# GloireLINVANI/3D_Gaussian_Splatting_Project

Hardware: AMD Instinct MI355X
Metric: Gaussians·views/sec labelled (3M G, 1080p), majority vote; first vote_view submit -> labels on the host (higher is better)
Workload: dtype f64

## Files before the change

### 3d_gaussian_splatting_project_amd/csrc/gsx_ctx.hpp

```cpp
#pragma once
#include <hip/hip_runtime.h>

#include <chrono>
#include <cstdarg>
#include <cstdint>
#include <cstdio>
#include <map>
#include <cstddef>
#include <string>
#include <vector>

#include "../../include/gsx.h"
#include "host_pack.hpp"

namespace gsx {

void set_global_error(const char* fmt, ...);
struct Ctx;
int fail(Ctx* c, int code, const char* fmt, ...);

#define GSX_HIP(ctx, call)                                                                         \
    do {                                                                                           \
        hipError_t e__ = (call);                                                                   \
        if (e__ != hipSuccess)                                                                     \
// ... 166 lines not shown
    long long compact_bytes = 0;
    void* h_labels = nullptr;
    size_t h_labels_cap = 0;
    hipEvent_t h_ev[kLabelChunks] = {nullptr, nullptr, nullptr, nullptr};
    void* h_views = nullptr;
    size_t h_views_cap = 0;
    hipEvent_t h_views_ev = nullptr;
    std::vector<ViewDesc> own_views;
    int own_first_view = 0;
    const void* pool_base = nullptr;
    int n_flushed = 0;
    bool planes_valid = false;
    bool planes_zero = false;
    bool planes_stale = false;
    DevBuf cnt, fv;
    DevBuf keys, labels;
    DevBuf labels8;
    DevBuf bcnt, bcodes;
    DevBuf cand, codes;
    bool labels_valid = false;
    int opt_filter_project = 1;
    int opt_early_vote = 1;
    int opt_early_at = 0;
    std::chrono::steady_clock::time_point early_t0;
    int opt_early_replay = 1;
    bool early_replayed = false;
    int early_state = 0;
    int early_done = 0;
    int early_batches = 0;
    hipStream_t stream2 = nullptr;
    bool stream_borrowed = false;
    int opt_render_share_stream = 1;
    bool early_inflight = false;
    hipEvent_t early_maps_ev = nullptr, early_done_ev = nullptr, early_up_ev = nullptr;
    DevBuf ecnt, efv;
    DevBuf erec;
    DevBuf e_views, e_cull;
    void* h_early = nullptr;
    size_t h_early_cap = 0;

    int64_t rn = 0;
    DevBuf r_order, r_buffer, r_tex;
    DevBuf r_sh;
    DevBuf r_fdc, r_shc;
    bool r_sh_valid = false, r_sh_on = false;
    int r_sh_deg = 0;
    DevBuf r_labels, r_edit_code, r_edit_tab, r_edit_hidden;
    bool r_edits_on = false;
    int64_t r_edit_hidden_n = 0;
    DevBuf r_image;
    int r_W = 0, r_H = 0;
    DevBuf r_ranges, r_small, r_scan;
    DevBuf r_depth, r_bucket, r_rect, r_count, r_offset, r_rec;
    DevBuf r_pre;
    struct PreSet {
        DevBuf depth, rect, rec, pre;
    };
    static constexpr int kPreSets = 3;
    PreSet r_sets[kPreSets];
    DevBuf r_pre_args;
    std::vector<unsigned long long> r_pre_args_host;
    hipEvent_t r_pre_ev[kPreSets] = {nullptr, nullptr, nullptr};
    int r_pre_ext = -1;
    int opt_render_multi_pre = 1;
    DevBuf r_keys0, r_keys1, r_vals0, r_vals1;
    DevBuf r_tile_order;
    int r_sorted_in = 0;
// ... 109 lines not shown
```

### 3d_gaussian_splatting_project_amd/csrc/vote.hip

```cpp
#include <hip/hip_runtime.h>

#include <chrono>
#include <cmath>

#include <algorithm>
#include <cmath>
#include <cstdlib>
#include <cstring>
#include <new>

#include <type_traits>

#ifndef GSX_ABLATE
#define GSX_ABLATE 0
#endif
#if GSX_ABLATE && !defined(GSX_EXPERIMENTS)
#error "GSX_ABLATE variants are experiments: build them with -DGSX_EXPERIMENTS (make experiments), never into libgsx.so"
#endif

#include "gsx_ctx.hpp"

namespace gsx {

static constexpr int kBlock = 256;
// ... 619 lines not shown
                    int c = old[u] + 1;
#pragma unroll
                    for (int w = 0; w < u; ++w) c += (bin[w] == bin[u]) ? 1 : 0;
                    h[bin[u]] = (uint8_t)c;
                    if (c >= bestc) {
                        bestc = c;
                        best = bin[u];
                    }
                }
            }
        } else {
#pragma unroll
            for (int u = 0; u < U; ++u) {
                if (bin[u] >= 0) {
                    const int c = h[bin[u]] + 1;
                    h[bin[u]] = (uint8_t)c;
                    if (c >= bestc) {
                        bestc = c;
                        best = bin[u];
                    }
                }
            }
        }
        };
    int vb = p.nviews;
    for (; vb >= U; vb -= U) chunk(std::true_type{}, vb);
    if (vb > 0) chunk(std::false_type{}, vb);
    if (valid) {
        const long long o = p.perm ? (long long)p.perm[i] : i;
        labels[o] = best - 1 + (best < 0);
    }
}

template <int U, int DIV>
__global__ __launch_bounds__(kBlock) void vote_record_kernel(FusedParams p, const ViewDesc* __restrict__ views,
                                                             uint8_t* __restrict__ rec) {
    const long long i = (long long)logical_block(blockIdx.x, gridDim.x, p.xcd_swizzle) * kBlock + threadIdx.x;
    const bool valid = i < p.n;
    const long long ic = valid ? i : 0;
    const float xf = p.x[ic], yf = p.y[ic], zf = p.z[ic];
    const double X = valid ? (double)xf : __builtin_nan("");
    const double Y = valid ? (double)yf : 0.0;
    const double Z = valid ? (double)zf : 0.0;
    const uint8_t* __restrict__ pool = p.pool;
    const int lane = threadIdx.x & 63;
    uint8_t* r = rec + (i - lane) * p.nviews + lane;
    const CullMasks cmask = wave_cull_masks(p.cull, p.cull_pitch, p.nviews, X, Y, Z, p.cull_tally);
    auto chunk = [&](auto full, int vb) {
        constexpr bool kFull = decltype(full)::value;
        int bin[U];
        gather_chunk<U, DIV, kFull>(views, pool, vb, X, Y, Z, cull_bits<U>(cmask, p.nviews - vb), bin, p.filt_h);
#pragma unroll
        for (int u = 0; u < U; ++u)
            if (kFull || vb - 1 - u >= 0) r[(vb - 1 - u) * 64] = (uint8_t)(bin[u] + 1);
    };
    int vb = p.nviews;
    for (; vb >= U; vb -= U) chunk(std::true_type{}, vb);
    if (vb > 0) chunk(std::false_type{}, vb);
}

template <int U, int DIV>
__global__ __launch_bounds__(kBlock) void vote_fused_replay_kernel(FusedParams p, const ViewDesc* __restrict__ views,
                                                                   const uint8_t* __restrict__ rec, int E,
                                                                   int* __restrict__ labels) {
    extern __shared__ uint32_t lds[];
    uint32_t* row = lds + threadIdx.x * p.stride_dw;
    uint8_t* h = reinterpret_cast<uint8_t*>(row);
    for (int k = 0; k < p.stride_dw; ++k) row[k] = 0;
    const long long i = (long long)logical_block(blockIdx.x, gridDim.x, p.xcd_swizzle) * kBlock + threadIdx.x;
    const bool valid = i < p.n;
    const long long ic = valid ? i : 0;
    const float xf = p.x[ic], yf = p.y[ic], zf = p.z[ic];
    const double X = valid ? (double)xf : __builtin_nan("");
    const double Y = valid ? (double)yf : 0.0;
    const double Z = valid ? (double)zf : 0.0;
    const uint8_t* __restrict__ pool = p.pool;
    int best = -1, bestc = 0;
    auto vote = [&](int b) {
        const int c = h[b] + 1;
        h[b] = (uint8_t)c;
        if (c >= bestc) {
            bestc = c;
            best = b;
        }
    };
    const CullMasks cmask = wave_cull_masks(p.cull, p.cull_pitch, p.nviews, X, Y, Z, p.cull_tally);
    auto chunk = [&](auto full, int vb) {
        constexpr bool kFull = decltype(full)::value;
        int bin[U];
        gather_chunk<U, DIV, kFull>(views, pool, vb, X, Y, Z, cull_bits<U>(cmask, p.nviews - vb), bin, p.filt_h);
#pragma unroll
        for (int u = 0; u < U; ++u)
            if (bin[u] >= 0) vote(bin[u]);
    };
    int vb = p.nviews;
    for (; vb >= U; vb -= U) chunk(std::true_type{}, vb);
    if (vb > 0) chunk(std::false_type{}, vb);
    constexpr int kReplay = 16;
    const int lane = threadIdx.x & 63;
    const uint8_t* __restrict__ r = rec + (i - lane) * E + lane;
    for (int v0 = E; v0 > 0; v0 -= kReplay) {
        unsigned b[kReplay];
#pragma unroll
        for (int j = 0; j < kReplay; ++j) {
            const int v = v0 - 1 - j;
            const unsigned got = r[max(v, 0) * 64];
            b[j] = v >= 0 ? got : 0u;
        }
#pragma unroll
        for (int j = 0; j < kReplay; ++j)
            if (b[j]) vote((int)b[j] - 1);
    }
    if (valid) {
        const long long o = p.perm ? (long long)p.perm[i] : i;
        labels[o] = best - 1 + (best < 0);
    }
}

typedef unsigned short u16x2 __attribute__((ext_vector_type(2)));
__device__ __forceinline__ uint32_t pk_max_u16(uint32_t a, uint32_t b) {
    return __builtin_bit_cast(uint32_t, __builtin_elementwise_max(__builtin_bit_cast(u16x2, a), __builtin_bit_cast(u16x2, b)));
}

template <int U, int DIV, int NQ>
__global__ __launch_bounds__(kBlock, 4) void vote_fused_final_kernel(FusedParams p, const ViewDesc* __restrict__ views,
                                                                     const uint8_t* __restrict__ cntA,
                                                                     const uint8_t* __restrict__ fvA,
                                                                     const uint8_t* __restrict__ recA, int E,
                                                                     int* __restrict__ labels, int ablate_arg) {
#ifdef GSX_EXPERIMENTS
    const int ablate = ablate_arg;
#else
    constexpr int ablate = 0;
#endif
    extern __shared__ uint32_t lds[];
    const long long i = (long long)logical_block(blockIdx.x, gridDim.x, p.xcd_swizzle) * kBlock + threadIdx.x;
    const bool valid = i < p.n;
    const long long ic = valid ? i : 0;
    const float xf = p.x[ic], yf = p.y[ic], zf = p.z[ic];
    const double X = valid ? (double)xf : __builtin_nan("");
    const double Y = valid ? (double)yf : 0.0;
    const double Z = valid ? (double)zf : 0.0;
    const uint8_t* __restrict__ pool = p.pool;
    const int lane = threadIdx.x & 63;
    const int g = lane >> 4;
    const int nq = (p.bins + 3) >> 2;
    uint32_t* wl = lds + (threadIdx.x >> 6) * (nq * 64);
// ... 492 lines not shown
    if (n_classes < 1 || n_classes > 255)
        return fail(c, GSX_E_UNSUPPORTED, "vote_begin: n_classes=%d outside [1,255] (u8 seg maps)", n_classes);
    if (first_view < 0 || total_views < 1 || total_views > 65535 || first_view >= total_views)
        return fail(c, GSX_E_INVALID, "vote_begin: first_view=%d total_views=%d (need 0 <= first < total <= 65535)",
                    first_view, total_views);
    GSX_HIP(c, hipSetDevice(c->device));
    c->n_classes = n_classes;
    c->bins = n_classes + 1;
    c->first_view = first_view;
    c->total_views = total_views;
    c->local_codes = c->opt_local_codes != 0;
    c->wide = total_views > 255 && !c->local_codes;
    c->slabs = c->opt_slabs > 0 ? c->opt_slabs : 1;
    c->sn = ((c->n + c->slabs - 1) / c->slabs + 255) / 256 * 256;
    if (c->sn == 0) c->sn = 256;
    c->n_pad = c->sn * c->slabs;
    c->views.clear();
    c->pend_count = 0;
    c->compact_bytes = 0;
    c->views_dirty = true;
    c->pool_base = nullptr;
    c->seg_used = 0;
    c->n_flushed = 0;
    c->planes_valid = false;
    c->planes_zero = false;
    c->planes_stale = false;
    c->labels_valid = false;
    {
        const int rcj = early_join(c);
        if (rcj) return rcj;
    }
    c->early_state = 0;
    c->early_done = 0;
    c->early_batches = 0;
    GSX_HIP(c, c->errflag.ensure(sizeof(int)));
    GSX_HIP(c, hipMemsetAsync(c->errflag.p, 0x7f, sizeof(int), c->stream));
    c->vote_begun = true;
    return GSX_OK;
}

static int pool_reserve(Ctx* c, size_t need) {
    if (need <= c->segpool.cap) return GSX_OK;
    {
        const int rcf = vote_flush_pending(c);
        if (rcf) return rcf;
    }
    if (c->early_state == 1 || c->early_batches > 0) {
        GSX_HIP(c, hipStreamSynchronize(c->stream2));
        c->early_inflight = false;
        c->early_state = -1;
        c->early_batches = 0;
    }
    size_t cap = c->segpool.cap ? c->segpool.cap : ((size_t)64 << 20);
    while (cap < need) cap *= 2;
    void* np = nullptr;
    GSX_HIP(c, hipMalloc(&np, cap));
    if (c->seg_used) {
        hipError_t e = hipMemcpyAsync(np, c->segpool.p, c->seg_used, hipMemcpyDeviceToDevice, c->stream);
        if (e == hipSuccess) e = hipStreamSynchronize(c->stream);
        if (e != hipSuccess) {
            (void)hipFree(np);
            return fail(c, GSX_E_HIP, "seg pool growth copy failed: %s", hipGetErrorString(e));
        }
    }
    c->segpool.release();
    c->segpool.p = np;
// ... 27 lines not shown
        const size_t all = stride * (size_t)(c->total_views - c->first_view);
        need = std::max(need, std::min(all, (size_t)32 << 30));
    }
    return pool_reserve(c, need);
}

static void push_view(Ctx* c, const gsx_camera* cam, const MapLayout& L, size_t off, int img_w, int img_h) {
    ViewDesc vd;
    fill_view_desc(vd, cam, L.w, L.h, img_w, img_h);
    vd.seg_off = (long long)off;
    vd.seg_row_bytes = L.strip_bytes;
    vd.coarse_row_bytes = L.cstrip_bytes;
    vd.coarse_delta = (unsigned)L.coarse_off;
    c->views.push_back(vd);
    c->views_dirty = true;
    c->seg_used = off + L.map_bytes;
    c->labels_valid = false;
}

static void launch_pack(Ctx* c, const PackArgs& a, int jobs, int seg_dtype, bool vec, long long cells);

static Workers* host_workers(Ctx* c, const void* near = nullptr) {
    if (!c->workers) {
        try {
            c->workers = new Workers(c->opt_host_threads > 0 ? c->opt_host_threads : default_host_threads(), numa_node_of(near));
        } catch (...) {
            c->workers = nullptr;
        }
    }
    return c->workers;
}

static int early_vote_stage(Ctx* c);

static int vote_view_host(Ctx* c, const gsx_camera* cam, const void* seg, int seg_dtype, int seg_w, int seg_h, int img_w, int img_h) {
    MapLayout L;
    int rc = view_prologue(c, "vote_view", cam, seg, 1, seg_dtype, seg_w, seg_h, img_w, img_h, L);
    if (rc) return rc;
    if (c->opt_host_pack) {
        const size_t stride = (L.map_bytes + 255) / 256 * 256;
        constexpr int kSlots = kDmaBatch * kDmaGroups;
        const bool compact = c->opt_host_compact && L.strip_bytes && L.cstrip_bytes;
        const CompactLayout CL = compact ? compact_layout(L) : CompactLayout{};
        const size_t slot_bytes = compact ? (CL.capacity + 255) / 256 * 256 : stride;
        if (c->hring_slot != slot_bytes || !c->hring || c->hring_compact != compact) {
            if ((rc = vote_flush_pending(c))) return rc;
            for (int g = 0; g < kDmaGroups; ++g) {
                if (c->hring_busy[g]) GSX_HIP(c, hipEventSynchronize(c->hring_ev[g]));
                c->hring_busy[g] = false;
                if (!c->hring_ev[g]) GSX_HIP(c, hipEventCreateWithFlags(&c->hring_ev[g], hipEventDisableTiming));
            }
            if (c->hring_bytes < slot_bytes * kSlots) {
                if (c->hring) GSX_HIP(c, hipHostFree(c->hring));
                c->hring = nullptr;
                c->hring_bytes = 0;
                GSX_HIP(c, hipHostMalloc(&c->hring, slot_bytes * kSlots, hipHostMallocDefault));
                c->hring_bytes = slot_bytes * kSlots;
            }
            if (!compact) std::memset(c->hring, 0, slot_bytes * kSlots);
            c->hring_slot = slot_bytes;
            c->hring_compact = compact;
            c->hring_next = 0;
            c->cgrp = 0;
            c->grp_recs = 0;
        }
        const size_t off = (c->seg_used + 255) / 256 * 256;
// ... 85 lines not shown
        const size_t raw = esz * (size_t)seg_w * (size_t)seg_h;
        if (slot.cap < raw) {
            GSX_HIP(c, hipHostFree(slot.p));
            slot.p = nullptr;
            slot.cap = 0;
            GSX_HIP(c, hipHostMalloc(&slot.p, raw, hipHostMallocDefault));
            slot.cap = raw;
        }
        DevBuf& land = c->dstage[c->ring_next];
        GSX_HIP(c, land.ensure(raw));
        host_copy(host_workers(c, seg), slot.p, seg, raw);
        GSX_HIP(c, hipMemcpyAsync(land.p, slot.p, raw, hipMemcpyHostToDevice, c->stream));
        const size_t off = (c->seg_used + 255) / 256 * 256;
        PackArgs a{};
        a.src[0] = land.p;
        a.dst[0] = c->segpool.as<uint8_t>() + off;
        a.view[0] = c->first_view + (int)c->views.size();
        a.w = L.w, a.h = L.h, a.strip_bytes = L.strip_bytes, a.cstrip_bytes = L.cstrip_bytes, a.cw = L.cw, a.ch = L.ch;
        a.bins = c->bins;
        a.coarse_off = (unsigned)L.coarse_off;
        a.err = c->errflag.as<int>();
        launch_pack(c, a, 1, seg_dtype, seg_w % 4 == 0, (long long)L.cw * L.ch);
        GSX_HIP(c, hipGetLastError());
        GSX_HIP(c, hipEventRecord(slot.ev, c->stream));
        slot.busy = true;
        c->ring_next = (c->ring_next + 1) % kPinSlots;
        push_view(c, cam, L, off, img_w, img_h);
        return GSX_OK;
    }
    return GSX_OK;
}

int vote_view(Ctx* c, const gsx_camera* cam, const void* seg, int seg_dtype, int seg_w, int seg_h, int img_w, int img_h) {
    const int rc = vote_view_host(c, cam, seg, seg_dtype, seg_w, seg_h, img_w, img_h);
    return rc ? rc : early_vote_stage(c);
}

static void launch_pack(Ctx* c, const PackArgs& a, int jobs, int seg_dtype, bool vec, long long cells) {
    using K = void (*)(PackArgs);
    static const K table[4][2] = {{seg_pack_fused_kernel<int32_t, 1, false>, seg_pack_fused_kernel<int32_t, 1, true>},
                                  {seg_pack_fused_kernel<int64_t, 1, false>, seg_pack_fused_kernel<int64_t, 1, true>},
                                  {seg_pack_fused_kernel<uint8_t, 0, false>, seg_pack_fused_kernel<uint8_t, 0, true>},
                                  {seg_pack_fused_kernel<uint8_t, 1, false>, seg_pack_fused_kernel<uint8_t, 1, true>}};
    ProfScope ps(c, "seg_pack");
    hipLaunchKernelGGL(table[seg_dtype][vec ? 1 : 0], dim3(grid_for(cells), jobs), dim3(kBlock), 0, c->stream, a);
}

int vote_views_device(Ctx* c, int n, const gsx_camera* cams, const void* const* segs, int seg_dtype, int seg_w, int seg_h,
                      int img_w, int img_h) {
    if (n <= 0) return n == 0 ? GSX_OK : fail(c, GSX_E_INVALID, "vote_views_device: n < 0");
    MapLayout L;
    int rc = view_prologue(c, "vote_views_device", cams, segs, n, seg_dtype, seg_w, seg_h, img_w, img_h, L);
    if (rc) return rc;
    for (int i = 0; i < n; ++i)
        if (!segs[i]) return fail(c, GSX_E_INVALID, "vote_views_device: map %d is NULL", i);
    const size_t esz = seg_dtype == GSX_SEG_I32 ? 4 : seg_dtype == GSX_SEG_I64 ? 8 : 1;
    const long long cells = (long long)L.cw * L.ch;
    for (int i0 = 0; i0 < n; i0 += kPackBatch) {
        const int m = std::min(kPackBatch, n - i0);
        PackArgs a{};
        bool vec = seg_w % 4 == 0;
        size_t off = 0;
        for (int k = 0; k < m; ++k) {
            off = (c->seg_used + 255) / 256 * 256;
            a.src[k] = segs[i0 + k];
            a.dst[k] = c->segpool.as<uint8_t>() + off;
            a.view[k] = c->first_view + (int)c->views.size();
            vec = vec && reinterpret_cast<uintptr_t>(segs[i0 + k]) % (4 * esz) == 0;
// ... 66 lines not shown
    }
    for (DevBuf& b : c->dstage) b.release();
    for (hipEvent_t& e : c->hring_ev) {
        if (e) (void)hipEventDestroy(e);
        e = nullptr;
    }
    if (c->hring) (void)hipHostFree(c->hring);
    c->hring = nullptr;
    c->hring_bytes = c->hring_slot = 0;
    std::free(c->h_scratch);
    c->h_scratch = nullptr;
    c->h_scratch_cap = 0;
    c->cstage.release();
    c->pend_count = 0;
    for (hipEvent_t& e : c->h_ev) {
        if (e) (void)hipEventDestroy(e);
        e = nullptr;
    }
    if (c->h_labels) (void)hipHostFree(c->h_labels);
    c->h_labels = nullptr;
    c->h_labels_cap = 0;
    if (c->h_views_ev) (void)hipEventDestroy(c->h_views_ev);
    c->h_views_ev = nullptr;
    if (c->h_views) (void)hipHostFree(c->h_views);
    c->h_views = nullptr;
    c->h_views_cap = 0;
    delete c->workers;
    c->workers = nullptr;
    if (c->stream2) {
        (void)hipStreamSynchronize(c->stream2);
        (void)hipStreamDestroy(c->stream2);
        c->stream2 = nullptr;
    }
    for (hipEvent_t* e : {&c->early_maps_ev, &c->early_done_ev, &c->early_up_ev}) {
        if (*e) (void)hipEventDestroy(*e);
        *e = nullptr;
    }
    if (c->h_early) (void)hipHostFree(c->h_early);
    c->h_early = nullptr;
    c->h_early_cap = 0;
    for (DevBuf* b : {&c->ecnt, &c->efv, &c->erec, &c->e_views, &c->e_cull}) b->release();
    c->early_state = -1;
}

int debug_host_pack(const void* seg, int seg_dtype, int w, int h, int n_classes, int tiled, int coarse, int threads,
                    uint8_t* out, int64_t out_cap, int64_t* bytes, int64_t* coarse_off, int32_t* bad) {
    if (!seg || w < 1 || h < 1 || w > 65535 || h > 65535 || n_classes < 1 || n_classes > 255 || seg_dtype < 0 || seg_dtype > 3)
        return fail(nullptr, GSX_E_INVALID, "debug_host_pack: bad arguments");
    const MapLayout L = map_layout(w, h, tiled != 0, coarse != 0 && n_classes + 1 <= 255);
    if (bytes) *bytes = (int64_t)L.map_bytes;
    if (coarse_off) *coarse_off = L.cstrip_bytes ? (int64_t)L.coarse_off : -1;
    if (!out) return GSX_OK;
    if (out_cap < (int64_t)L.map_bytes) return fail(nullptr, GSX_E_INVALID, "debug_host_pack: output buffer too small");
    Workers pool(threads > 0 ? threads : 1);
    const int b = host_pack_map(&pool, seg, seg_dtype, L, n_classes + 1, out);
    if (bad) *bad = b;
    return GSX_OK;
}

int debug_host_pack_compact(const void* seg, int seg_dtype, int w, int h, int n_classes, int threads, uint8_t* out, int64_t out_cap,
                            int64_t* bytes, int64_t* table_bytes, int64_t* stream_off, int32_t* bad) {
    if (!seg || w < 1 || h < 1 || w > 65535 || h > 65535 || n_classes < 1 || n_classes > 254 || seg_dtype < 0 || seg_dtype > 3 || !bytes)
        return fail(nullptr, GSX_E_INVALID, "debug_host_pack_compact: bad arguments");
    const MapLayout L = map_layout(w, h, true, true);
    const CompactLayout CL = compact_layout(L);
    if (table_bytes) *table_bytes = (int64_t)CL.table_bytes;
    if (stream_off) *stream_off = (int64_t)CL.stream_off;
    *bytes = (int64_t)CL.capacity;
    if (!out) return GSX_OK;
    if (out_cap < (int64_t)CL.capacity) return fail(nullptr, GSX_E_INVALID, "debug_host_pack_compact: output buffer too small");
    void* scratch = std::aligned_alloc(4096, (L.fine_bytes + 4095) / 4096 * 4096);
    if (!scratch) return fail(nullptr, GSX_E_HIP, "debug_host_pack_compact: out of memory");
    Workers pool(threads > 0 ? threads : 1);
    size_t blocks = 0;
// ... 228 lines not shown
static constexpr long long kEarlyMinGaussians = 1 << 18;
static constexpr int kEarlyMinViews = 32;
static constexpr double kEarlyUsPerGaussianView = 4.4e-6;
static constexpr double kRecordUsPerGaussianView = 1.7e-6;
static constexpr size_t kEarlySlack = 64 * 260;
static constexpr size_t kEarlyCullDoubles = (size_t)kCullStride * kCullPlanes * kEarlyPitch;

static bool early_common(const Ctx* c) {
    return c->opt_early_vote && c->first_view == 0 && !c->local_codes && c->slabs == 1 && c->n_flushed == 0 && !c->pool_base &&
           c->opt_flat_project && c->n > 0 && c->bins <= 255 &&
           (c->opt_early_vote == 2 || (c->n >= kEarlyMinGaussians && c->total_views >= kEarlyMinViews));
}
static bool early_possible(const Ctx* c) { return early_common(c) && c->total_views <= kMaxBatch && !c->wide; }
static bool early_batched_possible(const Ctx* c) { return early_common(c) && c->total_views > kMaxBatch && c->opt_batched_counts; }
static int early_batch_stage(Ctx* c);
static int early_batch_count(int total) {
    const int tail = std::min(std::max(total / 16, 16), 64), body = total - tail;
    return (body + kMaxBatch - 1) / kMaxBatch + 1;
}
static void early_batch_bounds(int total, int s, int& lo, int& hi) {
    const int tail = std::min(std::max(total / 16, 16), 64), body = total - tail;
    const int Sb = (body + kMaxBatch - 1) / kMaxBatch;
    if (s >= Sb) {
        lo = body;
        hi = total;
    } else {
        lo = (int)((long long)body * s / Sb);
        hi = (int)((long long)body * (s + 1) / Sb);
    }
}

static int early_upload(Ctx* c, int lo, int hi, int block, int blocks, hipStream_t st, int* dm) {
    const size_t vbytes = sizeof(ViewDesc) * kEarlyPitch, cbytes = sizeof(double) * kEarlyCullDoubles;
    if (!c->h_early) {
        GSX_HIP(c, hipHostMalloc(&c->h_early, vbytes + cbytes, hipHostMallocDefault));
        c->h_early_cap = vbytes + cbytes;
    }
    GSX_HIP(c, c->e_views.ensure(sizeof(ViewDesc) * (size_t)std::max(kEarlyPitch, c->total_views)));
    GSX_HIP(c, c->e_cull.ensure(cbytes * (size_t)std::max(2, blocks)));
    if (!c->early_up_ev) GSX_HIP(c, hipEventCreateWithFlags(&c->early_up_ev, hipEventDisableTiming));
    else GSX_HIP(c, hipEventSynchronize(c->early_up_ev));
    ViewDesc* hv = static_cast<ViewDesc*>(c->h_early);
    double* planes = reinterpret_cast<double*>(static_cast<char*>(c->h_early) + vbytes);
    std::memset(planes, 0, cbytes);
    const long long base = (long long)reinterpret_cast<uintptr_t>(c->segpool.p);
    bool simple = true, coarse = true;
    for (int i = lo; i < hi; ++i) {
        ViewDesc& v = hv[i - lo];
        v = c->views[i];
        v.seg_off += base;
        simple = simple && v.unit_scale && v.seg_row_bytes;
        coarse = coarse && v.coarse_row_bytes;
        double pl[kCullStride * kCullPlanes];
        cull_planes(v, pl);
        for (int k = 0; k < kCullStride * kCullPlanes; ++k) planes[(size_t)k * kEarlyPitch + (i - lo)] = pl[k];
    }
    *dm = !simple ? kDivFlat : (coarse && c->opt_seg_coarse ? (c->opt_filter_project ? kDivFiltCoarse : kDivFlatCoarse) : kDivFlatSimple);
    if (hi > lo) GSX_HIP(c, hipMemcpyAsync(c->e_views.as<ViewDesc>() + lo, hv, sizeof(ViewDesc) * (size_t)(hi - lo), hipMemcpyHostToDevice, st));
    GSX_HIP(c, hipMemcpyAsync(c->e_cull.as<double>() + (size_t)block * kEarlyCullDoubles, planes, cbytes, hipMemcpyHostToDevice, st));
    GSX_HIP(c, hipEventRecord(c->early_up_ev, st));
    return GSX_OK;
}

static FusedParams early_params(Ctx* c, int lo, int hi, int block, int stride_bytes_per_bin) {
    FusedParams p = fused_params(c, stride_bytes_per_bin);
    p.views = c->e_views.as<ViewDesc>() + lo;
    p.nviews = hi - lo;
    p.cull = c->opt_wave_cull ? c->e_cull.as<double>() + (size_t)block * kEarlyCullDoubles : nullptr;
    p.cull_pitch = kEarlyPitch;
    return p;
}

int early_join(Ctx* c) {
    if (!c->early_inflight) return GSX_OK;
    GSX_HIP(c, hipStreamWaitEvent(c->stream, c->early_done_ev, 0));
    c->early_inflight = false;
    return GSX_OK;
}

int second_stream(Ctx* c) {
    if (c->stream2) return GSX_OK;
    int least = 0, greatest = 0;
    GSX_HIP(c, hipDeviceGetStreamPriorityRange(&least, &greatest));
    GSX_HIP(c, hipStreamCreateWithPriority(&c->stream2, hipStreamNonBlocking, least));
    return GSX_OK;
}

static int early_streams(Ctx* c) {
    const int rc = second_stream(c);
    if (rc) return rc;
    if (!c->early_maps_ev) GSX_HIP(c, hipEventCreateWithFlags(&c->early_maps_ev, hipEventDisableTiming));
    if (!c->early_done_ev) GSX_HIP(c, hipEventCreateWithFlags(&c->early_done_ev, hipEventDisableTiming));
    return GSX_OK;
}

static int early_vote_stage(Ctx* c) {
    if (c->early_state == 0 && early_batched_possible(c)) return early_batch_stage(c);
    if (c->early_state != 0 || !early_possible(c)) return GSX_OK;
    const int nv = (int)c->views.size();
    int at;
    if (c->opt_early_at > 0) {
        at = std::max(1, (int)(((long long)c->total_views * c->opt_early_at + 999) / 1000));
        if (nv != at) return GSX_OK;
    } else {
        const auto now = std::chrono::steady_clock::now();
        if (nv == 1) c->early_t0 = now;
        if (nv < std::max(8, c->total_views / 4)) return GSX_OK;
        const double t_map = std::chrono::duration<double, std::micro>(now - c->early_t0).count() / (double)(nv - 1);
        const double t_view = (c->opt_early_replay ? kRecordUsPerGaussianView : kEarlyUsPerGaussianView) * (double)c->n;
        const int lo = (c->total_views + 1) / 2, hi = (int)(((long long)c->total_views * 880) / 1000);
        const int want = std::min(std::max((int)std::ceil(c->total_views * t_map / (t_map + t_view)), lo), std::max(lo, hi));
        if (nv < want) return GSX_OK;
        at = nv;
    }
    if (at >= c->total_views) return GSX_OK;
    int rc = vote_flush_pending(c);
    if (rc) return rc;
    if ((rc = early_streams(c))) return rc;
    const size_t plane = (size_t)c->bins * (size_t)c->n_pad;
    if (!c->opt_early_replay) {
        GSX_HIP(c, c->ecnt.ensure(plane + kEarlySlack));
        GSX_HIP(c, c->efv.ensure(plane + kEarlySlack));
    }
    GSX_HIP(c, c->erec.ensure((size_t)c->n_pad * (size_t)at));
    if ((rc = ensure_tally(c))) return rc;
    GSX_HIP(c, hipEventRecord(c->early_maps_ev, c->stream));
    GSX_HIP(c, hipStreamWaitEvent(c->stream2, c->early_maps_ev, 0));
    int dm = kDivFlat;
    if ((rc = early_upload(c, 0, at, 0, 2, c->stream2, &dm))) return rc;
    if (c->opt_early_replay) {
        FusedParams p = early_params(c, 0, at, 0, 1);
        auto kr = dm == kDivFiltCoarse ? vote_record_kernel<kUnroll, kDivFiltCoarse>
                 : dm == kDivFlatCoarse ? vote_record_kernel<kUnroll, kDivFlatCoarse>
                  : dm == kDivFlatSimple ? vote_record_kernel<kUnroll, kDivFlatSimple>
                                         : vote_record_kernel<kUnroll, kDivFlat>;
        {
            ProfScope ps(c, "vote_early_record", c->stream2);
            hipLaunchKernelGGL(kr, dim3(grid_for(c->n)), dim3(kBlock), 0, c->stream2, p, p.views, c->erec.as<uint8_t>());
            GSX_HIP(c, hipGetLastError());
        }
        GSX_HIP(c, hipEventRecord(c->early_done_ev, c->stream2));
        c->early_inflight = true;
        c->early_done = at;
        c->early_state = 1;
        c->early_replayed = true;
        return GSX_OK;
    }
    c->early_replayed = false;
    FusedParams p = early_params(c, 0, at, 0, 2);
    const size_t lds = (size_t)kBlock * p.stride_dw * 4;
    auto k = dm == kDivFiltCoarse ? vote_fused_planes_kernel<kUnroll, uint8_t, kDivFiltCoarse>
                 : dm == kDivFlatCoarse ? vote_fused_planes_kernel<kUnroll, uint8_t, kDivFlatCoarse>
             : dm == kDivFlatSimple ? vote_fused_planes_kernel<kUnroll, uint8_t, kDivFlatSimple>
                                    : vote_fused_planes_kernel<kUnroll, uint8_t, kDivFlat>;
    if ((rc = set_lds(c, k, lds))) return rc;
    {
        ProfScope ps(c, "vote_early_planes", c->stream2);
        hipLaunchKernelGGL(k, dim3(grid_for(c->n)), dim3(kBlock), lds, c->stream2, p, p.views, c->ecnt.as<uint8_t>(), c->efv.as<uint8_t>(),
                           64LL, 0, 1, 0, c->erec.as<uint8_t>());
        GSX_HIP(c, hipGetLastError());
    }
    GSX_HIP(c, hipEventRecord(c->early_done_ev, c->stream2));
    c->early_inflight = true;
    c->early_done = at;
    c->early_state = 1;
    return GSX_OK;
}

static int early_batch_stage(Ctx* c) {
    const int nv = (int)c->views.size();
    const int S = early_batch_count(c->total_views);
    const int s = c->early_batches;
    if (s >= S - 1) return GSX_OK;
// ... 4 lines not shown
    if (rc) return rc;
    if ((rc = early_streams(c))) return rc;
    const size_t plane = (size_t)c->bins * (size_t)c->n_pad;
    GSX_HIP(c, c->bcnt.ensure(plane * S));
    if ((rc = ensure_tally(c))) return rc;
    GSX_HIP(c, hipEventRecord(c->early_maps_ev, c->stream));
    GSX_HIP(c, hipStreamWaitEvent(c->stream2, c->early_maps_ev, 0));
    int dm = kDivFlat;
    if ((rc = early_upload(c, lo, hi, s, S, c->stream2, &dm))) return rc;
    FusedParams p = early_params(c, lo, hi, s, 1);
    const size_t lds = (size_t)kBlock * p.stride_dw * 4;
    auto k = dm == kDivFiltCoarse ? vote_fused_counts_kernel<kUnroll, kDivFiltCoarse>
                 : dm == kDivFlatCoarse ? vote_fused_counts_kernel<kUnroll, kDivFlatCoarse>
             : dm == kDivFlatSimple ? vote_fused_counts_kernel<kUnroll, kDivFlatSimple>
                                    : vote_fused_counts_kernel<kUnroll, kDivFlat>;
    if ((rc = set_lds(c, k, lds))) return rc;
    {
        ProfScope ps(c, "vote_early_counts", c->stream2);
        hipLaunchKernelGGL(k, dim3(grid_for(c->n)), dim3(kBlock), lds, c->stream2, p, p.views, c->bcnt.as<uint8_t>() + plane * s, (long long)c->n_pad);
        GSX_HIP(c, hipGetLastError());
    }
    GSX_HIP(c, hipEventRecord(c->early_done_ev, c->stream2));
    c->early_inflight = true;
    c->early_batches = s + 1;
    c->early_done = hi;
    return GSX_OK;
}

static int early_vote_finish(Ctx* c) {
    const int nv = (int)c->views.size();
    int rc = vote_flush_pending(c);
    if (rc) return rc;
    int dm = kDivFlat;
    if ((rc = early_upload(c, c->early_done, nv, 1, 2, c->stream, &dm))) return rc;
    GSX_HIP(c, c->labels.ensure(sizeof(int) * (size_t)(c->n_pad ? c->n_pad : 1)));
    if (c->early_replayed) {
        FusedParams pr = early_params(c, c->early_done, nv, 1, 1);
        const size_t ldsr = (size_t)kBlock * pr.stride_dw * 4;
        auto kr = dm == kDivFiltCoarse ? vote_fused_replay_kernel<kUnroll, kDivFiltCoarse>
                 : dm == kDivFlatCoarse ? vote_fused_replay_kernel<kUnroll, kDivFlatCoarse>
                  : dm == kDivFlatSimple ? vote_fused_replay_kernel<kUnroll, kDivFlatSimple>
                                         : vote_fused_replay_kernel<kUnroll, kDivFlat>;
        if ((rc = set_lds(c, kr, ldsr))) return rc;
        if ((rc = early_join(c))) return rc;
        if ((c->opt_ablate >> 4) & 2) pr.nviews = 0;
        ProfScope ps(c, "vote_fused_replay");
        hipLaunchKernelGGL(kr, dim3(grid_for(c->n)), dim3(kBlock), ldsr, c->stream, pr, pr.views, c->erec.as<uint8_t>(), c->early_done,
                           c->labels.as<int>());
        GSX_HIP(c, hipGetLastError());
        return GSX_OK;
    }
    FusedParams p = early_params(c, c->early_done, nv, 1, 1);
    const size_t lds = (size_t)(kBlock / 64) * ((c->bins + 3) / 4) * 256;
    constexpr int kRegRows = 38;
    const bool regs = c->bins <= 4 * kRegRows;
    auto k = dm == kDivFiltCoarse ? (regs ? vote_fused_final_kernel<kUnroll, kDivFiltCoarse, kRegRows> : vote_fused_final_kernel<kUnroll, kDivFiltCoarse, 0>)
                 : dm == kDivFlatCoarse ? (regs ? vote_fused_final_kernel<kUnroll, kDivFlatCoarse, kRegRows> : vote_fused_final_kernel<kUnroll, kDivFlatCoarse, 0>)
             : dm == kDivFlatSimple ? (regs ? vote_fused_final_kernel<kUnroll, kDivFlatSimple, kRegRows> : vote_fused_final_kernel<kUnroll, kDivFlatSimple, 0>)
                                    : (regs ? vote_fused_final_kernel<kUnroll, kDivFlat, kRegRows> : vote_fused_final_kernel<kUnroll, kDivFlat, 0>);
    if ((rc = set_lds(c, k, lds))) return rc;
    if ((rc = early_join(c))) return rc;
    const int ablate = (c->opt_ablate >> 4) & 63;
    if (ablate & 2) p.nviews = 0;
    ProfScope ps(c, "vote_fused_final");
    hipLaunchKernelGGL(k, dim3(grid_for(c->n)), dim3(kBlock), lds, c->stream, p, p.views, c->ecnt.as<uint8_t>(), c->efv.as<uint8_t>(),
                       c->erec.as<uint8_t>(), c->early_done, c->labels.as<int>(), ablate);
    GSX_HIP(c, hipGetLastError());
    return GSX_OK;
}

int vote_flush(Ctx* c) {
    if (!c->vote_begun) return fail(c, GSX_E_STATE, "vote_flush before vote_begin");
    GSX_HIP(c, hipSetDevice(c->device));
    int rc = early_join(c);
    if (rc) return rc;
    if ((rc = sync_views(c))) return rc;
    rc = ensure_planes(c);
    if (rc) return rc;
    const int nv = (int)c->views.size();
    if (c->n <= 0 || c->n_flushed >= nv) {
        c->n_flushed = nv;
        return clear_stale_planes(c);
    }
    FusedParams p{};
// ... 255 lines not shown
    {
        ProfScope ps(c, "vote_tie_resolve");
        hipLaunchKernelGGL(vote_tie_resolve_kernel, dim3(grid_for(npad)), dim3(kBlock), 0, c->stream, c->bcodes.as<uint16_t>(), S, npad,
                           c->keys.as<int>());
    }
    GSX_HIP(c, hipGetLastError());
    return GSX_OK;
}

static int labels_for_range(Ctx* c, const VoteRange& r, bool to_sorted) {
    int rc = early_join(c);
    if (rc) return rc;
    if ((rc = sync_views(c))) return rc;
    GSX_HIP(c, c->keys.ensure(sizeof(int) * (size_t)(c->n_pad ? c->n_pad : 1)));
    GSX_HIP(c, c->labels.ensure(sizeof(int) * (size_t)(c->n_pad ? c->n_pad : 1)));
    const uint32_t* perm = c->sorted ? c->perm.as<uint32_t>() : nullptr;
    if ((int)c->views.size() <= kMaxBatch)
        return labels_one_batch(c, r, to_sorted ? nullptr : perm, to_sorted ? c->keys.as<int>() : c->labels.as<int>());
    if ((rc = labels_batched(c, r))) return rc;
    if (!to_sorted && r.n > 0) {
        ProfScope ps(c, "vote_labels");
        hipLaunchKernelGGL(unpermute_labels_kernel, dim3(grid_for(r.n)), dim3(kBlock), 0, c->stream, c->keys.as<int>(), r.n, perm,
                           c->labels.as<int>());
        GSX_HIP(c, hipGetLastError());
    }
    return GSX_OK;
}

int vote_finalize(Ctx* c, int32_t* labels_out) {
    if (!c->vote_begun) return fail(c, GSX_E_STATE, "vote_finalize before vote_begin");
    GSX_HIP(c, hipSetDevice(c->device));
    const int nv = (int)c->views.size();
    const bool batched_ok = !c->local_codes && c->opt_batched_counts;
    if (c->early_state == 1 && early_possible(c) && nv >= c->early_done && nv <= kMaxBatch) {
        int rc = early_vote_finish(c);
        if (rc) return rc;
        return labels_to_host(c, labels_out);
    }
    if (c->n_flushed == 0 && (nv <= kMaxBatch || batched_ok)) {
        int rc = labels_for_range(c, VoteRange{0, c->n}, false);
        if (rc) return rc;
        return labels_to_host(c, labels_out);
    }
    int rc = vote_flush(c);
    if (rc) return rc;
    if ((rc = vote_tiebreak_keys(c))) return rc;
    return vote_labels_from_keys(c, labels_out);
}

int vote_export(Ctx* c, int64_t reserve_bytes, void* blobs_out, void** pool_dev, int64_t* pool_bytes) {
    if (!c->vote_begun) return fail(c, GSX_E_STATE, "vote_export before vote_begin");
    if (c->pool_base) return fail(c, GSX_E_STATE, "vote_export after vote_import");
    GSX_HIP(c, hipSetDevice(c->device));
    if (reserve_bytes < 0) return fail(c, GSX_E_INVALID, "vote_export: negative size");
    {
        const int rcf = vote_flush_pending(c);
        if (rcf) return rcf;
    }
    const size_t used = (c->seg_used + 255) / 256 * 256;
    int rc = pool_reserve(c, std::max<size_t>(std::max<size_t>((size_t)reserve_bytes, used), 256));
    if (rc) return rc;
    c->views_dirty = true;
    static_assert(sizeof(ViewDesc) == GSX_VIEW_BLOB_BYTES, "view blob size is part of the ABI");
    if (blobs_out && !c->views.empty()) std::memcpy(blobs_out, c->views.data(), sizeof(ViewDesc) * c->views.size());
    if (pool_dev) *pool_dev = c->segpool.p;
    if (pool_bytes) *pool_bytes = (int64_t)used;
    return GSX_OK;
// ... 312 lines not shown
```

Baseline: 90.50 billion.

## Add late record stage and mask-driven replay kernel for early voting

Early voting now records per-view bins for all views in up to three staged record kernels, including a late stage that runs on the secondary stream while the last views are still being submitted. Each record pass also writes per-wave bitmasks of views that produced any vote. The final step becomes a pure replay kernel: it reads only the recorded views flagged in the masks, builds a compact per-wave view list in LDS, and prefetches bytes in double-buffered groups of 32, instead of recomputing projections for the remaining views. Upload staging gets three rotating pinned host slots with their own events so uploads need not wait on each other. The cost is a larger record buffer sized for every view, plus extra mask traffic and more complex finalize conditions.

New measurement: 90.28 billion. No clear change (-0.2%).

```diff
diff --git a/3d_gaussian_splatting_project_amd/csrc/gsx_ctx.hpp b/3d_gaussian_splatting_project_amd/csrc/gsx_ctx.hpp
--- a/3d_gaussian_splatting_project_amd/csrc/gsx_ctx.hpp
+++ b/3d_gaussian_splatting_project_amd/csrc/gsx_ctx.hpp
@@ -222,7 +222,11 @@
     bool stream_borrowed = false;
     int opt_render_share_stream = 1;
     bool early_inflight = false;
-    hipEvent_t early_maps_ev = nullptr, early_done_ev = nullptr, early_up_ev = nullptr;
+    hipEvent_t early_maps_ev = nullptr, early_done_ev = nullptr;
+    hipEvent_t early_up_ev[3] = {nullptr, nullptr, nullptr};
+    int early_recorded = 0;
+    int early_stages = 0;
+    DevBuf emask;
     DevBuf ecnt, efv;
     DevBuf erec;
     DevBuf e_views, e_cull;
diff --git a/3d_gaussian_splatting_project_amd/csrc/vote.hip b/3d_gaussian_splatting_project_amd/csrc/vote.hip
--- a/3d_gaussian_splatting_project_amd/csrc/vote.hip
+++ b/3d_gaussian_splatting_project_amd/csrc/vote.hip
@@ -675,9 +675,11 @@
     }
 }
 
+static constexpr int kMaskWords = 4;
 template <int U, int DIV>
 __global__ __launch_bounds__(kBlock) void vote_record_kernel(FusedParams p, const ViewDesc* __restrict__ views,
-                                                             uint8_t* __restrict__ rec) {
+                                                             uint8_t* __restrict__ rec, int pitch, int view0,
+                                                             unsigned long long* __restrict__ mask) {
     const long long i = (long long)logical_block(blockIdx.x, gridDim.x, p.xcd_swizzle) * kBlock + threadIdx.x;
     const bool valid = i < p.n;
     const long long ic = valid ? i : 0;
@@ -687,75 +689,118 @@
     const double Z = valid ? (double)zf : 0.0;
     const uint8_t* __restrict__ pool = p.pool;
     const int lane = threadIdx.x & 63;
-    uint8_t* r = rec + (i - lane) * p.nviews + lane;
+    uint8_t* r = rec + (i - lane) * pitch + (long long)view0 * 64 + lane;
     const CullMasks cmask = wave_cull_masks(p.cull, p.cull_pitch, p.nviews, X, Y, Z, p.cull_tally);
+    unsigned long long any[kMaskWords] = {0, 0, 0, 0};
     auto chunk = [&](auto full, int vb) {
         constexpr bool kFull = decltype(full)::value;
         int bin[U];
         gather_chunk<U, DIV, kFull>(views, pool, vb, X, Y, Z, cull_bits<U>(cmask, p.nviews - vb), bin, p.filt_h);
-#pragma unroll
-        for (int u = 0; u < U; ++u)
-            if (kFull || vb - 1 - u >= 0) r[(vb - 1 - u) * 64] = (uint8_t)(bin[u] + 1);
+        unsigned cb = 0;
+#pragma unroll
+        for (int u = 0; u < U; ++u) {
+            if (kFull || vb - 1 - u >= 0) {
+                r[(vb - 1 - u) * 64] = (uint8_t)(bin[u] + 1);
+                cb |= __builtin_amdgcn_ballot_w64(bin[u] >= 0) ? 1u << (U - 1 - u) : 0u;
+            }
+        }
+        const int g = view0 + (kFull ? vb - U : 0);
+        if (!kFull) cb >>= U - vb;
+        const int w0 = g >> 6, sh = g & 63;
+        const unsigned long long lo = (unsigned long long)cb << sh, hi = sh > 64 - U ? (unsigned long long)cb >> (64 - sh) : 0ull;
+#pragma unroll
+        for (int w = 0; w < kMaskWords; ++w) any[w] |= (w == w0 ? lo : 0ull) | (w == w0 + 1 ? hi : 0ull);
     };
     int vb = p.nviews;
     for (; vb >= U; vb -= U) chunk(std::true_type{}, vb);
     if (vb > 0) chunk(std::false_type{}, vb);
-}
-
-template <int U, int DIV>
-__global__ __launch_bounds__(kBlock) void vote_fused_replay_kernel(FusedParams p, const ViewDesc* __restrict__ views,
-                                                                   const uint8_t* __restrict__ rec, int E,
-                                                                   int* __restrict__ labels) {
+    if (lane == 0) {
+        unsigned long long* m = mask + ((i - lane) >> 6) * kMaskWords;
+#pragma unroll
+        for (int w = 0; w < kMaskWords; ++w) m[w] = any[w];
+    }
+}
+
+__global__ __launch_bounds__(kBlock) void vote_replay_kernel(long long n, int bins, int xcd_swizzle, const uint32_t* __restrict__ perm,
+                                                             const uint8_t* __restrict__ rec, int pitch,
+                                                             const unsigned long long* __restrict__ masks, long long mask_stride,
+                                                             int nmasks, int* __restrict__ labels) {
     extern __shared__ uint32_t lds[];
-    uint32_t* row = lds + threadIdx.x * p.stride_dw;
-    uint8_t* h = reinterpret_cast<uint8_t*>(row);
-    for (int k = 0; k < p.stride_dw; ++k) row[k] = 0;
-    const long long i = (long long)logical_block(blockIdx.x, gridDim.x, p.xcd_swizzle) * kBlock + threadIdx.x;
-    const bool valid = i < p.n;
-    const long long ic = valid ? i : 0;
-    const float xf = p.x[ic], yf = p.y[ic], zf = p.z[ic];
-    const double X = valid ? (double)xf : __builtin_nan("");
-    const double Y = valid ? (double)yf : 0.0;
-    const double Z = valid ? (double)zf : 0.0;
-    const uint8_t* __restrict__ pool = p.pool;
+    const int lane = threadIdx.x & 63;
+    const int nq = (bins + 3) >> 2;
+    uint32_t* wbase = lds + (threadIdx.x >> 6) * ((nq + 1) * 64);
+    uint8_t* list = reinterpret_cast<uint8_t*>(wbase);
+    uint32_t* col = wbase + 64 + lane;
+    wbase[lane] = 0;
+    for (int q = 0; q < nq; ++q) col[q * 64] = 0;
+    uint8_t* h = reinterpret_cast<uint8_t*>(col);
+    const long long i = (long long)logical_block(blockIdx.x, gridDim.x, xcd_swizzle) * kBlock + threadIdx.x;
+    const long long wave = (i - lane) >> 6;
+    unsigned long long mine = 0;
+    if (lane < kMaskWords * nmasks) mine = masks[(lane >> 2) * mask_stride + wave * kMaskWords + (lane & 3)];
+    const unsigned mlo = (unsigned)mine, mhi = (unsigned)(mine >> 32);
+    auto word = [&](int w) {
+        unsigned lo = 0, hi = 0;
+#pragma unroll
+        for (int s = 0; s < 3; ++s) {
+            lo |= (unsigned)__builtin_amdgcn_readlane((int)mlo, 4 * s + w);
+            hi |= (unsigned)__builtin_amdgcn_readlane((int)mhi, 4 * s + w);
+        }
+        return ((unsigned long long)hi << 32) | lo;
+    };
+    const unsigned long long m0 = word(0), m1 = word(1), m2 = word(2), m3 = word(3);
+    const int c3 = __builtin_popcountll(m3), c2 = __builtin_popcountll(m2), c1 = __builtin_popcountll(m1), c0 = __builtin_popcountll(m0);
+    const int nv = c3 + c2 + c1 + c0;
+    auto put = [&](unsigned long long m, int w, int before) {
+        if ((m >> lane) & 1ull) list[before + __builtin_popcountll((m >> 1) >> lane)] = (uint8_t)(64 * w + lane);
+    };
+    put(m3, 3, 0);
+    put(m2, 2, c3);
+    put(m1, 1, c3 + c2);
+    put(m0, 0, c3 + c2 + c1);
+    __atomic_signal_fence(__ATOMIC_SEQ_CST);
+    __builtin_amdgcn_wave_barrier();
     int best = -1, bestc = 0;
-    auto vote = [&](int b) {
-        const int c = h[b] + 1;
-        h[b] = (uint8_t)c;
-        if (c >= bestc) {
-            bestc = c;
-            best = b;
+    constexpr int kReplay = 32;
+    const uint8_t* __restrict__ r = rec + (i - lane) * pitch + lane;
+    auto load = [&](unsigned (&b)[kReplay], int k0) {
+        const uint4* lp = reinterpret_cast<const uint4*>(list + k0);
+#pragma unroll
+        for (int q = 0; q < kReplay / 16; ++q) {
+            const uint4 w4 = lp[q];
+            const unsigned w[4] = {w4.x, w4.y, w4.z, w4.w};
+#pragma unroll
+            for (int j = 0; j < 16; ++j) b[16 * q + j] = r[((w[j >> 2] >> (8 * (j & 3))) & 255u) * 64u];
         }
     };
-    const CullMasks cmask = wave_cull_masks(p.cull, p.cull_pitch, p.nviews, X, Y, Z, p.cull_tally);
-    auto chunk = [&](auto full, int vb) {
-        constexpr bool kFull = decltype(full)::value;
-        int bin[U];
-        gather_chunk<U, DIV, kFull>(views, pool, vb, X, Y, Z, cull_bits<U>(cmask, p.nviews - vb), bin, p.filt_h);
-#pragma unroll
-        for (int u = 0; u < U; ++u)
-            if (bin[u] >= 0) vote(bin[u]);
+    auto apply = [&](const unsigned (&b)[kReplay], int cnt) {
+#pragma unroll
+        for (int j = 0; j < kReplay; ++j) {
+            if (j < cnt && b[j]) {
+                const int bin = (int)b[j] - 1;
+                uint8_t* cp = h + ((bin >> 2) << 8) + (bin & 3);
+                const int c = *cp + 1;
+                *cp = (uint8_t)c;
+                if (c >= bestc) {
+                    bestc = c;
+                    best = bin;
+                }
+            }
+        }
     };
-    int vb = p.nviews;
-    for (; vb >= U; vb -= U) chunk(std::true_type{}, vb);
-    if (vb > 0) chunk(std::false_type{}, vb);
-    constexpr int kReplay = 16;
-    const int lane = threadIdx.x & 63;
-    const uint8_t* __restrict__ r = rec + (i - lane) * E + lane;
-    for (int v0 = E; v0 > 0; v0 -= kReplay) {
-        unsigned b[kReplay];
-#pragma unroll
-        for (int j = 0; j < kReplay; ++j) {
-            const int v = v0 - 1 - j;
-            const unsigned got = r[max(v, 0) * 64];
-            b[j] = v >= 0 ? got : 0u;
-        }
-#pragma unroll
-        for (int j = 0; j < kReplay; ++j)
-            if (b[j]) vote((int)b[j] - 1);
-    }
-    if (valid) {
-        const long long o = p.perm ? (long long)p.perm[i] : i;
+    unsigned cur[kReplay], nxt[kReplay];
+    int k0 = 0;
+    load(cur, 0);
+    while (k0 + kReplay < nv) {
+        load(nxt, k0 + kReplay);
+        apply(cur, kReplay);
+#pragma unroll
+        for (int j = 0; j < kReplay; ++j) cur[j] = nxt[j];
+        k0 += kReplay;
+    }
+    apply(cur, nv - k0);
+    if (i < n) {
+        const long long o = perm ? (long long)perm[i] : i;
         labels[o] = best - 1 + (best < 0);
     }
 }
@@ -1314,6 +1359,8 @@
     }
     c->early_state = 0;
     c->early_done = 0;
+    c->early_recorded = 0;
+    c->early_stages = 0;
     c->early_batches = 0;
     GSX_HIP(c, c->errflag.ensure(sizeof(int)));
     GSX_HIP(c, hipMemsetAsync(c->errflag.p, 0x7f, sizeof(int), c->stream));
@@ -1407,6 +1454,7 @@
 }
 
 static int early_vote_stage(Ctx* c);
+static int early_late_stage(Ctx* c);
 
 static int vote_view_host(Ctx* c, const gsx_camera* cam, const void* seg, int seg_dtype, int seg_w, int seg_h, int img_w, int img_h) {
     MapLayout L;
@@ -1558,8 +1606,9 @@
 }
 
 int vote_view(Ctx* c, const gsx_camera* cam, const void* seg, int seg_dtype, int seg_w, int seg_h, int img_w, int img_h) {
-    const int rc = vote_view_host(c, cam, seg, seg_dtype, seg_w, seg_h, img_w, img_h);
-    return rc ? rc : early_vote_stage(c);
+    int rc = vote_view_host(c, cam, seg, seg_dtype, seg_w, seg_h, img_w, img_h);
+    if (rc || (rc = early_vote_stage(c))) return rc;
+    return early_late_stage(c);
 }
 
 static void launch_pack(Ctx* c, const PackArgs& a, int jobs, int seg_dtype, bool vec, long long cells) {
@@ -1692,14 +1741,14 @@
         (void)hipStreamDestroy(c->stream2);
         c->stream2 = nullptr;
     }
-    for (hipEvent_t* e : {&c->early_maps_ev, &c->early_done_ev, &c->early_up_ev}) {
+    for (hipEvent_t* e : {&c->early_maps_ev, &c->early_done_ev, &c->early_up_ev[0], &c->early_up_ev[1], &c->early_up_ev[2]}) {
         if (*e) (void)hipEventDestroy(*e);
         *e = nullptr;
     }
     if (c->h_early) (void)hipHostFree(c->h_early);
     c->h_early = nullptr;
     c->h_early_cap = 0;
-    for (DevBuf* b : {&c->ecnt, &c->efv, &c->erec, &c->e_views, &c->e_cull}) b->release();
+    for (DevBuf* b : {&c->ecnt, &c->efv, &c->erec, &c->emask, &c->e_views, &c->e_cull}) b->release();
     c->early_state = -1;
 }
 
@@ -1994,16 +2043,19 @@
 
 static int early_upload(Ctx* c, int lo, int hi, int block, int blocks, hipStream_t st, int* dm) {
     const size_t vbytes = sizeof(ViewDesc) * kEarlyPitch, cbytes = sizeof(double) * kEarlyCullDoubles;
+    constexpr int kSlots = 3;
+    const int slot = block % kSlots;
     if (!c->h_early) {
-        GSX_HIP(c, hipHostMalloc(&c->h_early, vbytes + cbytes, hipHostMallocDefault));
-        c->h_early_cap = vbytes + cbytes;
+        GSX_HIP(c, hipHostMalloc(&c->h_early, kSlots * (vbytes + cbytes), hipHostMallocDefault));
+        c->h_early_cap = kSlots * (vbytes + cbytes);
     }
     GSX_HIP(c, c->e_views.ensure(sizeof(ViewDesc) * (size_t)std::max(kEarlyPitch, c->total_views)));
-    GSX_HIP(c, c->e_cull.ensure(cbytes * (size_t)std::max(2, blocks)));
-    if (!c->early_up_ev) GSX_HIP(c, hipEventCreateWithFlags(&c->early_up_ev, hipEventDisableTiming));
-    else GSX_HIP(c, hipEventSynchronize(c->early_up_ev));
-    ViewDesc* hv = static_cast<ViewDesc*>(c->h_early);
-    double* planes = reinterpret_cast<double*>(static_cast<char*>(c->h_early) + vbytes);
+    GSX_HIP(c, c->e_cull.ensure(cbytes * (size_t)std::max(3, blocks)));
+    if (!c->early_up_ev[slot]) GSX_HIP(c, hipEventCreateWithFlags(&c->early_up_ev[slot], hipEventDisableTiming));
+    else GSX_HIP(c, hipEventSynchronize(c->early_up_ev[slot]));
+    char* stage = static_cast<char*>(c->h_early) + (size_t)slot * (vbytes + cbytes);
+    ViewDesc* hv = reinterpret_cast<ViewDesc*>(stage);
+    double* planes = reinterpret_cast<double*>(stage + vbytes);
     std::memset(planes, 0, cbytes);
     const long long base = (long long)reinterpret_cast<uintptr_t>(c->segpool.p);
     bool simple = true, coarse = true;
@@ -2020,7 +2072,7 @@
     *dm = !simple ? kDivFlat : (coarse && c->opt_seg_coarse ? (c->opt_filter_project ? kDivFiltCoarse : kDivFlatCoarse) : kDivFlatSimple);
     if (hi > lo) GSX_HIP(c, hipMemcpyAsync(c->e_views.as<ViewDesc>() + lo, hv, sizeof(ViewDesc) * (size_t)(hi - lo), hipMemcpyHostToDevice, st));
     GSX_HIP(c, hipMemcpyAsync(c->e_cull.as<double>() + (size_t)block * kEarlyCullDoubles, planes, cbytes, hipMemcpyHostToDevice, st));
-    GSX_HIP(c, hipEventRecord(c->early_up_ev, st));
+    GSX_HIP(c, hipEventRecord(c->early_up_ev[slot], st));
     return GSX_OK;
 }
 
@@ -2053,6 +2105,43 @@
     if (rc) return rc;
     if (!c->early_maps_ev) GSX_HIP(c, hipEventCreateWithFlags(&c->early_maps_ev, hipEventDisableTiming));
     if (!c->early_done_ev) GSX_HIP(c, hipEventCreateWithFlags(&c->early_done_ev, hipEventDisableTiming));
+    return GSX_OK;
+}
+
+static constexpr int kRecordStages = 3;
+static constexpr int kLateTail = kDmaBatch;
+static constexpr int kLateMinViews = 8;
+
+static int launch_record(Ctx* c, int lo, int hi, int block, int dm, const char* name, hipStream_t st) {
+    FusedParams p = early_params(c, lo, hi, block, 1);
+    auto kr = dm == kDivFiltCoarse ? vote_record_kernel<kUnroll, kDivFiltCoarse>
+             : dm == kDivFlatCoarse ? vote_record_kernel<kUnroll, kDivFlatCoarse>
+              : dm == kDivFlatSimple ? vote_record_kernel<kUnroll, kDivFlatSimple>
+                                     : vote_record_kernel<kUnroll, kDivFlat>;
+    unsigned long long* mask = c->emask.as<unsigned long long>() + (size_t)c->early_stages * kMaskWords * (size_t)(c->n_pad / 64);
+    {
+        ProfScope ps(c, name, st);
+        hipLaunchKernelGGL(kr, dim3(grid_for(c->n)), dim3(kBlock), 0, st, p, p.views, c->erec.as<uint8_t>(), c->total_views, lo, mask);
+        GSX_HIP(c, hipGetLastError());
+    }
+    c->early_recorded = hi;
+    ++c->early_stages;
+    return GSX_OK;
+}
+
+static int early_late_stage(Ctx* c) {
+    if (c->early_state != 1 || !c->early_replayed || c->early_stages != 1 || !early_possible(c)) return GSX_OK;
+    const int nv = (int)c->views.size();
+    if (nv != c->total_views - kLateTail || nv - c->early_recorded < kLateMinViews) return GSX_OK;
+    int rc = vote_flush_pending(c);
+    if (rc) return rc;
+    GSX_HIP(c, hipEventRecord(c->early_maps_ev, c->stream));
+    GSX_HIP(c, hipStreamWaitEvent(c->stream2, c->early_maps_ev, 0));
+    int dm = kDivFlat;
+    if ((rc = early_upload(c, c->early_recorded, nv, 1, kRecordStages, c->stream2, &dm))) return rc;
+    if ((rc = launch_record(c, c->early_recorded, nv, 1, dm, "vote_late_record", c->stream2))) return rc;
+    GSX_HIP(c, hipEventRecord(c->early_done_ev, c->stream2));
+    c->early_inflight = true;
     return GSX_OK;
 }
 
@@ -2084,23 +2173,15 @@
         GSX_HIP(c, c->ecnt.ensure(plane + kEarlySlack));
         GSX_HIP(c, c->efv.ensure(plane + kEarlySlack));
     }
-    GSX_HIP(c, c->erec.ensure((size_t)c->n_pad * (size_t)at));
+    GSX_HIP(c, c->erec.ensure((size_t)c->n_pad * (size_t)(c->opt_early_replay ? c->total_views : at)));
+    if (c->opt_early_replay) GSX_HIP(c, c->emask.ensure(sizeof(unsigned long long) * kMaskWords * kRecordStages * (size_t)(c->n_pad / 64)));
     if ((rc = ensure_tally(c))) return rc;
     GSX_HIP(c, hipEventRecord(c->early_maps_ev, c->stream));
     GSX_HIP(c, hipStreamWaitEvent(c->stream2, c->early_maps_ev, 0));
     int dm = kDivFlat;
-    if ((rc = early_upload(c, 0, at, 0, 2, c->stream2, &dm))) return rc;
+    if ((rc = early_upload(c, 0, at, 0, kRecordStages, c->stream2, &dm))) return rc;
     if (c->opt_early_replay) {
-        FusedParams p = early_params(c, 0, at, 0, 1);
-        auto kr = dm == kDivFiltCoarse ? vote_record_kernel<kUnroll, kDivFiltCoarse>
-                 : dm == kDivFlatCoarse ? vote_record_kernel<kUnroll, kDivFlatCoarse>
-                  : dm == kDivFlatSimple ? vote_record_kernel<kUnroll, kDivFlatSimple>
-                                         : vote_record_kernel<kUnroll, kDivFlat>;
-        {
-            ProfScope ps(c, "vote_early_record", c->stream2);
-            hipLaunchKernelGGL(kr, dim3(grid_for(c->n)), dim3(kBlock), 0, c->stream2, p, p.views, c->erec.as<uint8_t>());
-            GSX_HIP(c, hipGetLastError());
-        }
+        if ((rc = launch_record(c, 0, at, 0, dm, "vote_early_record", c->stream2))) return rc;
         GSX_HIP(c, hipEventRecord(c->early_done_ev, c->stream2));
         c->early_inflight = true;
         c->early_done = at;
@@ -2171,24 +2252,24 @@
     int rc = vote_flush_pending(c);
     if (rc) return rc;
     int dm = kDivFlat;
-    if ((rc = early_upload(c, c->early_done, nv, 1, 2, c->stream, &dm))) return rc;
     GSX_HIP(c, c->labels.ensure(sizeof(int) * (size_t)(c->n_pad ? c->n_pad : 1)));
     if (c->early_replayed) {
-        FusedParams pr = early_params(c, c->early_done, nv, 1, 1);
-        const size_t ldsr = (size_t)kBlock * pr.stride_dw * 4;
-        auto kr = dm == kDivFiltCoarse ? vote_fused_replay_kernel<kUnroll, kDivFiltCoarse>
-                 : dm == kDivFlatCoarse ? vote_fused_replay_kernel<kUnroll, kDivFlatCoarse>
-                  : dm == kDivFlatSimple ? vote_fused_replay_kernel<kUnroll, kDivFlatSimple>
-                                         : vote_fused_replay_kernel<kUnroll, kDivFlat>;
-        if ((rc = set_lds(c, kr, ldsr))) return rc;
+        if (nv > c->early_recorded) {
+            const int block = c->early_stages;
+            if ((rc = early_upload(c, c->early_recorded, nv, block, kRecordStages, c->stream, &dm))) return rc;
+            if ((rc = launch_record(c, c->early_recorded, nv, block, dm, "vote_late_record", c->stream))) return rc;
+        }
+        const size_t ldsr = (size_t)(kBlock / 64) * ((c->bins + 3) / 4 + 1) * 256;
+        if ((rc = set_lds(c, vote_replay_kernel, ldsr))) return rc;
         if ((rc = early_join(c))) return rc;
-        if ((c->opt_ablate >> 4) & 2) pr.nviews = 0;
         ProfScope ps(c, "vote_fused_replay");
-        hipLaunchKernelGGL(kr, dim3(grid_for(c->n)), dim3(kBlock), ldsr, c->stream, pr, pr.views, c->erec.as<uint8_t>(), c->early_done,
-                           c->labels.as<int>());
+        hipLaunchKernelGGL(vote_replay_kernel, dim3(grid_for(c->n)), dim3(kBlock), ldsr, c->stream, (long long)c->n, c->bins, c->opt_xcd_swizzle,
+                           c->sorted ? c->perm.as<uint32_t>() : nullptr, c->erec.as<uint8_t>(), c->total_views,
+                           c->emask.as<unsigned long long>(), (long long)kMaskWords * (c->n_pad / 64), c->early_stages, c->labels.as<int>());
         GSX_HIP(c, hipGetLastError());
         return GSX_OK;
     }
+    if ((rc = early_upload(c, c->early_done, nv, 1, 2, c->stream, &dm))) return rc;
     FusedParams p = early_params(c, c->early_done, nv, 1, 1);
     const size_t lds = (size_t)(kBlock / 64) * ((c->bins + 3) / 4) * 256;
     constexpr int kRegRows = 38;
@@ -2510,7 +2591,8 @@
     GSX_HIP(c, hipSetDevice(c->device));
     const int nv = (int)c->views.size();
     const bool batched_ok = !c->local_codes && c->opt_batched_counts;
-    if (c->early_state == 1 && early_possible(c) && nv >= c->early_done && nv <= kMaxBatch) {
+    const bool stages_left = !c->early_replayed || nv == c->early_recorded || c->early_stages < kRecordStages;
+    if (c->early_state == 1 && early_possible(c) && nv >= std::max(c->early_done, c->early_recorded) && nv <= kMaxBatch && stages_left) {
         int rc = early_vote_finish(c);
         if (rc) return rc;
         return labels_to_host(c, labels_out);
```
